# hwwang55/GraphGAN

Hardware: AMD Instinct MI355X
Metric: sampled_edges_per_sec (higher is better)
Workload: dtype f32

## Files before the change

### graphgan_amd/csrc/gg_api.hip

```cpp
#include <stdarg.h>
#include <stdlib.h>
#include <string.h>
#include <sys/stat.h>
#include <unistd.h>

#include <algorithm>
#include <atomic>
#include <thread>

#include "gg_internal.h"

namespace gg {

thread_local std::string g_last_error;

int fail(gg_ctx *ctx, int code, const char *fmt, ...) {
    char buf[1024];
    va_list ap;
    va_start(ap, fmt);
    vsnprintf(buf, sizeof(buf), fmt, ap);
    va_end(ap);
    g_last_error = buf;
    if (ctx) ctx->err = buf;
    return code;
// ... 329 lines not shown
    hipDeviceProp_t prop;
    GG_HIP(nullptr, hipGetDeviceProperties(&prop, cfg->device));
    if (strncmp(prop.gcnArchName, "gfx950", 6) != 0)
        return fail(nullptr, GG_EHIP, "gg_create: device %d is %s; kernels are built for gfx950 only", cfg->device, prop.gcnArchName);
    GG_HIP(nullptr, hipSetDevice(cfg->device));

    gg_ctx *ctx = new gg_ctx();
    ctx->n_node = n_node;
    ctx->n_emb = n_emb;
    ctx->ld = (n_emb + 3) / 4 * 4;
    ctx->cfg = *cfg;
    ctx->device = cfg->device;
    ctx->n_cus = prop.multiProcessorCount > 0 ? prop.multiProcessorCount : 256;
    if (const char *lv = getenv("GG_WALK_LEVELS")) ctx->walk_levels = atoi(lv);
    if (const char *pe = getenv("GG_PROFILE_EVERY")) ctx->profile_every = std::max(0, atoi(pe));
    if (const char *fw = getenv("GG_COMM_FAKE_WORLD")) ctx->fake_world = atoi(fw);
    if (const char *ow = getenv("GG_COMM_OWNER")) ctx->owner_exchange = atoi(ow);
    if (const char *bf = getenv("GG_COMM_BF16")) ctx->comm_bf16 = atoi(bf) != 0;
    if (const char *om = getenv("GG_COMM_OWNER_MIN")) ctx->owner_min_bound = atoll(om);
    if (const char *dt = getenv("GG_DETERMINISTIC")) ctx->deterministic = atoi(dt) != 0;
    if (const char *nc = getenv("GG_NO_DIST_CACHE")) ctx->dc_enabled = atoi(nc) == 0;
    if (const char *ft = getenv("GG_FIN_THRESHOLD")) ctx->fin_threshold = std::max(0, atoi(ft));
    if (const char *st = getenv("GG_STAGE_T")) ctx->sg_threshold = std::max(0, atoi(st));
    if (const char *ws = getenv("GG_WALK_SPLIT")) ctx->split_enabled = atoi(ws) != 0;
    if (const char *em = getenv("GG_ES_MODE")) ctx->es_mode = std::min(2, std::max(0, atoi(em)));
    if (const char *er = getenv("GG_ES_RATIO")) ctx->es_ratio_num = std::max(1, atoi(er));
    if (const char *eh = getenv("GG_ES_HUB")) ctx->es_hub = std::max(0, atoi(eh));
    if (const char *wm = getenv("GG_WALK_SPLIT_MIN")) ctx->split_min_walks = std::max(512, atoi(wm));
    for (auto &m : ctx->alive_prof) for (auto &v : m) v = -1;
    if (const char *dr = getenv("GG_COMM_DENSE_RATIO")) ctx->dense_exchange_ratio = (float)atof(dr);
#define GG_TRY(call)                        \
    do {                                    \
        int rc__ = (call);                  \
        if (rc__ != GG_OK) {                \
            g_last_error = ctx->err;        \
            gg_destroy(ctx);                \
            return rc__;                    \
        }                                   \
    } while (0)
    auto body = [&]() -> int {
        GG_HIP(ctx, hipStreamCreateWithFlags(&ctx->stream, hipStreamNonBlocking));
        {
            int lo = 0, hi = 0;
            const char *wp = getenv("GG_WALK_PRIORITY");
            if (wp && atoi(wp) != 0 && hipDeviceGetStreamPriorityRange(&lo, &hi) == hipSuccess && hi != lo)
                GG_HIP(ctx, hipStreamCreateWithPriority(&ctx->stream2, hipStreamNonBlocking, atoi(wp) > 0 ? hi : lo));
// ... 62 lines not shown
    return GG_OK;
}

int gg_destroy(gg_ctx *ctx) {
    if (!ctx) return GG_OK;
    (void)hipSetDevice(ctx->device);
    if (ctx->stream) (void)hipStreamSynchronize(ctx->stream);
    if (ctx->stream2) (void)hipStreamSynchronize(ctx->stream2);
    comm_destroy(ctx);
    for (int m = 0; m < 2; ++m) {
        Model &M = ctx->model[m];
        float *ps[] = {M.E, M.b, M.mE, M.vE, M.mb, M.vb};
        for (float *p : ps)
            if (p) (void)hipFree(p);
    }
    void *ps[] = {ctx->gradE, ctx->gradb, ctx->touched, ctx->touched_list, ctx->touched_cnt, ctx->g_rowptr, ctx->g_col, ctx->dev_ctr,
                  ctx->es, ctx->es_stamp, ctx->g_rev};
    for (void *p : ps)
        if (p) (void)hipFree(p);
    free_trees(ctx);
    DevBuf *bufs[] = {&ctx->w_slots_m[0], &ctx->w_slots_m[1], &ctx->w_ptr_m[0], &ctx->w_ptr_m[1], &ctx->w_samples, &ctx->w_paths, &ctx->w_len, &ctx->w_status,
                      &ctx->w_first, &ctx->w_abort, &ctx->w_scratch, &ctx->d_center, &ctx->d_neighbor, &ctx->d_label, &ctx->d_cnt,
                      &ctx->d_ptr, &ctx->g_node1, &ctx->g_node2, &ctx->g_reward, &ctx->g_cnt, &ctx->g_ptr, &ctx->scan_tmp,
                      &ctx->step_u, &ctx->step_v, &ctx->step_x, &ctx->sg_cnt, &ctx->sg_off, &ctx->sg_slot, &ctx->sg_list, &ctx->sg_rows, &ctx->sg_bias, &ctx->sg_tot, &ctx->sg_key, &ctx->touched_ptr, &ctx->x_cnt, &ctx->x_send_ids, &ctx->x_send_rows,
                      &ctx->x_recv_ids, &ctx->x_recv_rows, &ctx->x_nglob, &ctx->x_own, &ctx->st_item, &ctx->st_item2, &ctx->st_cur, &ctx->st_prev, &ctx->st_len,
                      &ctx->st_alive, &ctx->st_rank, &ctx->bfs_key, &ctx->bfs_bm, &ctx->bfs_misc, &ctx->bfs_sparse, &ctx->bfs_rowptr32, &ctx->lv_pfx, &ctx->dc_keys, &ctx->dc_vals, &ctx->dc_words, &ctx->lv_beg, &ctx->lv_k, &ctx->lv_chunks, &ctx->lv_coff, &ctx->lv_scores, &ctx->lv_chunk_owner, &ctx->lv_prefix, &ctx->lv_big, &ctx->lv_fe, &ctx->fin_list, &ctx->table_bad, &ctx->sgp_cnt, &ctx->sgp_off, &ctx->sgp_slot, &ctx->sgp_list, &ctx->sgp_tot, &ctx->sgp_key, &ctx->sgp_scan, &ctx->sgp_hub, &ctx->sg_hub, &ctx->hub_acc,
                      &ctx->q3_store, &ctx->q3s_off, &ctx->ep_center, &ctx->ep_neighbor, &ctx->ep_label, &ctx->ep_node1, &ctx->ep_node2, &ctx->ep_reward, &ctx->topk_adj,
                      &ctx->gs_es, &ctx->gs_cpre, &ctx->pt_starts, &ctx->pt_paths, &ctx->pt_len, &ctx->pt_cnt, &ctx->pt_ptr, &ctx->pt_noise, &ctx->pt_sample};
    for (DevBuf *b : bufs) b->release();
    for (hipEvent_t e : ctx->lv_ev)
        if (e) (void)hipEventDestroy(e);
    for (auto &tr : ctx->tm_ev)
        for (hipEvent_t e : tr)
            if (e) (void)hipEventDestroy(e);
    for (hipEvent_t e : ctx->pt_ev)
        if (e) (void)hipEventDestroy(e);
    if (ctx->h_pin) (void)hipHostFree(ctx->h_pin);
    for (hipEvent_t e : {ctx->ev_walk_done, ctx->ev_slots_done, ctx->ev_gen_pass, ctx->ev_main_mark, ctx->ev_fork, ctx->ev_join, ctx->ev_score[0], ctx->ev_score[1]})
        if (e) (void)hipEventDestroy(e);
    if (ctx->stream3) {
        (void)hipStreamSynchronize(ctx->stream3);
        (void)hipStreamDestroy(ctx->stream3);
    }
    if (ctx->stream2) {
        (void)hipStreamSynchronize(ctx->stream2);
        (void)hipStreamDestroy(ctx->stream2);
    }
// ... 673 lines not shown
```

### graphgan_amd/csrc/gg_internal.h

```cpp
#pragma once
#include <hip/hip_runtime.h>
#include <stdint.h>
#include <stdio.h>
#include <string>
#include <vector>

#include "../../include/graphgan_hip.h"

namespace gg {

struct DevBuf {
    void *p = nullptr;
    size_t bytes = 0;
    hipError_t reserve(size_t need) {
        if (need <= bytes) return hipSuccess;
        if (p) {
            (void)hipDeviceSynchronize();
            (void)hipFree(p);
        }
        p = nullptr;
        bytes = 0;
        size_t want = need + need / 4 + 256;
        hipError_t e = hipMalloc(&p, want);
        if (e == hipSuccess) bytes = want;
// ... 137 lines not shown
    gg::DevBuf d_center, d_neighbor, d_label, d_cnt, d_ptr;
    int64_t d_rows = 0;
    gg::DevBuf g_node1, g_node2, g_reward, g_cnt, g_ptr;
    int64_t g_pairs = 0;
    bool g_paths_valid = false;
    bool g_begun = false;
    struct { int32_t n_slots = 0, n_sample = 0; uint64_t seed = 0; uint32_t stream = 0; } g_begun_args;
    gg::DevBuf touched_ptr;
    gg::DevBuf bfs_key, bfs_bm, bfs_misc, bfs_sparse, bfs_rowptr32;
    bool bfs_rowptr32_valid = false;
    gg::DevBuf q3_store, q3s_off;
    int64_t q3_words = 0;
    bool q3_store_ready = false;
    gg::DevBuf ep_center, ep_neighbor, ep_label, ep_node1, ep_node2, ep_reward;
    int64_t ep_rows = 0, ep_pairs = 0;
    std::vector<int32_t> ep_slots;
    bool in_epoch_add = false;
    int n_cus = 256;
    gg::DevBuf scan_tmp, step_u, step_v, step_x;
    gg::DevBuf sg_cnt, sg_off, sg_slot, sg_list, sg_rows, sg_bias, sg_tot, sg_key;
    bool g_pairs_filled = false;
    bool sg_cnt_dirty = false;
    gg::DevBuf sgp_cnt, sgp_off, sgp_slot, sgp_list, sgp_tot, sgp_key, sgp_scan, sgp_hub;
    gg::DevBuf sg_hub, hub_acc;
    int64_t hub_cap = 0;
    hipEvent_t ev_slots_done = nullptr;
    bool g_slots_ready = false;
    bool sgp_cnt_clean = false;
    int g_slots_unused = 0;
    int64_t g_slots_walks = 0;
    int32_t g_slots_stride = 0;
    int32_t *sg_cnt_active = nullptr;
    bool sg_active = false;
    int sg_threshold = 64;

    unsigned long long *dev_ctr = nullptr;
    gg_counters ctr{};

    void *comm = nullptr;
    bool comm_rsag = true;
    size_t grad_elems_padded = 0;
    int64_t d_rows_max = 0, g_pairs_max = 0;
    int64_t step_bound = 0;
    int64_t comm_steps_sparse = 0, comm_steps_dense = 0, comm_bytes_sent = 0;
    int32_t rank = 0, world = 1;
    bool deterministic = true;
    float dense_exchange_ratio = 1.5f;
    int32_t fake_world = 0;
    gg::DevBuf x_cnt, x_send_ids, x_send_rows, x_recv_ids, x_recv_rows;
    gg::DevBuf x_nglob;
    gg::DevBuf x_own;
    int32_t owner_exchange = 1;
    bool comm_bf16 = false;
    int64_t owner_min_bound = 4096;
    int64_t comm_steps_owner = 0;

// ... 88 lines not shown
```

### graphgan_amd/csrc/steps.hip

```cpp
#include <stdlib.h>

#include <algorithm>
#include <cmath>
#include <vector>

#include "gg_internal.h"

namespace gg {

struct HubAcc {
    unsigned long long *acc;
    int64_t cap;
    float scale;
};
__device__ __forceinline__ unsigned long long *hub_row(const HubAcc &h, int slot, int ld) {
    const int64_t k = -3 - (int64_t)slot;
    return (slot <= -3 && k < h.cap) ? h.acc + k * (ld + 1) : nullptr;
}
__device__ __forceinline__ void hub_add(unsigned long long *p, float x, float scale) {
    atomicAdd(p, (unsigned long long)__float2ll_rn(x * scale));
}

struct StepArgs {
    float *E, *b;
    float *gE, *gb;
    int32_t *touched, *touched_list, *touched_cnt;
    int ld, track;
    const int32_t *u, *v;
    const float *x;
    int n;
    float lambda, inv_n;
    const int64_t *n_glob;
    int is_d;
    int ppg;
    unsigned long long *prof;
    const int32_t *slot_v, *slot_u;
    float *stage, *stage_b;
    HubAcc hub;
};

__global__ __launch_bounds__(256) void pair_occ_count_kernel(const int32_t *u, const int32_t *v, int n, int ppg, int32_t *cnt,
                                                             int32_t *slot_v, int32_t *slot_u) {
    const int p = blockIdx.x * blockDim.x + threadIdx.x;
    if (p >= n) return;
    slot_v[p] = atomicAdd(&cnt[v[p]], 1);
    const bool run_end = p == n - 1 || (p + 1) % ppg == 0 || u[p + 1] != u[p];
    slot_u[p] = run_end ? atomicAdd(&cnt[u[p]], 1) : -2;
}

__global__ __launch_bounds__(256) void pair_occ_slot_kernel(const int32_t *u, const int32_t *v, int n, const int32_t *cnt, const int32_t *off,
                                                            int T, int32_t *slot_v, int32_t *slot_u, int32_t *key) {
    const int p = blockIdx.x * blockDim.x + threadIdx.x;
    if (p >= n) return;
    const int iv = v[p], iu = u[p];
    const int sv = cnt[iv] <= T ? off[iv] + slot_v[p] : -3 - off[iv];
    slot_v[p] = sv;
    if (sv >= 0) key[sv] = 2 * p + 1;
    if (slot_u[p] != -2) {
        const int su = cnt[iu] <= T ? off[iu] + slot_u[p] : -3 - off[iu];
        slot_u[p] = su;
        if (su >= 0) key[su] = 2 * p;
    }
// ... 74 lines not shown
        for (int i = 0; i < NF; ++i) {
            const int f = t + 16 * i;
            if (f < a.ld) {
                const float x = fu[f], y = fv[f];
                accu[i] += ds * y + a.lambda * x;
                const float gval = ds * x + a.lambda * y;
                if (st) gv[f] = gval;
                else atomicAdd(gv + f, gval);
            }
        }
        if (t == 0) {
            const float gbv = a.is_d ? ds + a.lambda * bv : ds;
            if (st) {
                a.stage_b[slv] = gbv;
            } else {
                atomicAdd(a.gb + iv, gbv);
                if (a.track) a.touched[iv] = 1;
            }
        }
    }
    flush_u(p1 - 1);
}

template <int NF, bool STAGED>
__global__ __launch_bounds__(256) void pair_grad16_kernel(const StepArgs a) {
    const int t = threadIdx.x & 15;
    const int64_t g = ((int64_t)blockIdx.x * blockDim.x + threadIdx.x) >> 4;
    const int64_t p0 = g * 16;
    if (p0 >= a.n) return;
    const int np = (int)min((int64_t)16, (int64_t)a.n - p0);
    const float inv_n = a.n_glob ? 1.0f / (float)(*a.n_glob) : a.inv_n;
    const bool mine = t < np;
    const int myu = mine ? a.u[p0 + t] : 0, myv = mine ? a.v[p0 + t] : 0;
    const float myx = mine ? a.x[p0 + t] : 0.f;
    const int my_sv = (STAGED && mine) ? a.slot_v[p0 + t] : -1;
    const int my_su = (STAGED && mine) ? a.slot_u[p0 + t] : -1;
    const float mybv = a.b[myv];
    const int nextu = __shfl(myu, (t + 1) & 15, 16);
    const bool my_end = mine && (t == np - 1 || nextu != myu);
    auto fetch = [&](int j, float (&ru)[NF], float (&rv)[NF]) {
        const int jj = j < np ? j : 0;
        const float *su = a.E + (int64_t)__shfl(myu, jj, 16) * a.ld, *sv = a.E + (int64_t)__shfl(myv, jj, 16) * a.ld;
#pragma unroll
        for (int i = 0; i < NF; ++i) {
            const int f = t + 16 * i;
            const int fc = f < a.ld ? f : a.ld - 1;
            ru[i] = su[fc];
            rv[i] = sv[fc];
        }
    };
    float U[3][NF], V[3][NF], accu[NF];
#pragma unroll
    for (int i = 0; i < NF; ++i) accu[i] = 0.f;
    fetch(0, U[0], V[0]);
    fetch(1, U[1], V[1]);
#pragma unroll 1
    for (int j0 = 0; j0 < np; j0 += 3) {
#pragma unroll
        for (int r = 0; r < 3; ++r) {
            const int j = j0 + r;
            if (j >= np) break;
            fetch(j + 2, U[(r + 2) % 3], V[(r + 2) % 3]);
// ... 9 lines not shown
            acc += __shfl_xor(acc, 4, 64);
            acc += __shfl_xor(acc, 2, 64);
            acc += __shfl_xor(acc, 1, 64);
            const float bv = __shfl(mybv, j, 16), xj = __shfl(myx, j, 16);
            const float s = acc + bv;
            const float sg = 1.0f / (1.0f + expf(-s));
            float ds;
            if (a.is_d) {
                ds = sg - xj;
            } else {
                const bool inside = (sg >= 1e-5f) && (sg <= 1.0f);
                ds = inside ? -(xj * inv_n) * (1.0f - sg) : 0.0f;
            }
            const int iv = __shfl(myv, j, 16), iu = __shfl(myu, j, 16);
            const int slv = __shfl(my_sv, j, 16), slu = __shfl(my_su, j, 16);
            const bool st = STAGED && slv >= 0;
            unsigned long long *hv = STAGED && !st ? hub_row(a.hub, slv, a.ld) : nullptr;
            float *gv = st ? a.stage + (int64_t)slv * a.ld : a.gE + (int64_t)iv * a.ld;
#pragma unroll
            for (int i = 0; i < NF; ++i) {
                const int f = t + 16 * i;
                if (f < a.ld) {
                    accu[i] += ds * V[r][i] + a.lambda * U[r][i];
                    const float gval = ds * U[r][i] + a.lambda * V[r][i];
                    if (st) gv[f] = gval;
                    else if (STAGED && hv) hub_add(hv + f, gval, a.hub.scale);
                    else atomicAdd(gv + f, gval);
                }
            }
            if (t == 0) {
                const float gbv = a.is_d ? ds + a.lambda * bv : ds;
                if (st) {
                    a.stage_b[slv] = gbv;
                } else {
                    if (STAGED && hv) hub_add(hv + a.ld, gbv, a.hub.scale);
                    else atomicAdd(a.gb + iv, gbv);
                    if (a.track) a.touched[iv] = 1;
                }
            }
            if (__shfl((int)my_end, j, 16)) {
                if (STAGED && slu >= 0) {
                    float *gu = a.stage + (int64_t)slu * a.ld;
#pragma unroll
                    for (int i = 0; i < NF; ++i) {
                        const int f = t + 16 * i;
                        if (f < a.ld) gu[f] = accu[i];
                    }
                    if (t == 0) a.stage_b[slu] = 0.f;
                } else {
                    float *gu = a.gE + (int64_t)iu * a.ld;
                    unsigned long long *hu = STAGED ? hub_row(a.hub, slu, a.ld) : nullptr;
#pragma unroll
                    for (int i = 0; i < NF; ++i) {
                        const int f = t + 16 * i;
                        if (f < a.ld) {
                            if (STAGED && hu) hub_add(hu + f, accu[i], a.hub.scale);
                            else atomicAdd(gu + f, accu[i]);
                        }
                    }
                    if (t == 0 && a.track) a.touched[iu] = 1;
                }
#pragma unroll
                for (int i = 0; i < NF; ++i) accu[i] = 0.f;
            }
        }
    }
}

struct PathArgs {
    float *E, *b, *gE, *gb;
    int32_t *touched, *touched_list, *touched_cnt;
// ... 206 lines not shown
#pragma unroll
            for (int i = 0; i < NF; ++i) { R[sl][i] = R[sl + 1][i]; A[sl][i] = A[sl + 1][i]; }
        }
        enter(2, Rq[0], qnode[0], qslot[0], qbv[0]);
        qnode[0] = qnode[1]; qbv[0] = qbv[1]; qslot[0] = qslot[1];
#pragma unroll
        for (int i = 0; i < NF; ++i) Rq[0][i] = Rq[1][i];
    }
}

struct OptArgs {
    float *E, *b, *mE, *vE, *mb, *vb, *gE, *gb;
    const int64_t *touched_ptr;
    const int64_t *touched_total;
    int64_t nE;
    int n_node, ld;
    float lr_t, b1, b2, eps, lr;
    int32_t *touched, *touched_list, *touched_cnt;
    int32_t *sg_cnt;
    const int4 *sg_list;
    const int64_t *sg_tot;
    const float *stage, *stage_b;
    const int32_t *stage_key;
    unsigned long long *bad;
};

__device__ __forceinline__ bool nonfinite4(const float4 &x) { return !(__builtin_isfinite(x.x) && __builtin_isfinite(x.y) && __builtin_isfinite(x.z) && __builtin_isfinite(x.w)); }

__device__ __forceinline__ void adam_elem(float &var, float &m, float &v, float g, const OptArgs &a) {
    m = m * a.b1;
    m = m + (1.0f - a.b1) * g;
    v = v * a.b2;
    v = v + (g * g) * (1.0f - a.b2);
    var = var - (a.lr_t * m) / (sqrtf(v) + a.eps);
}

__global__ __launch_bounds__(256) void adam_dense_kernel(const OptArgs a) {
    const int64_t n4 = a.nE >> 2;
    const int64_t stride = (int64_t)gridDim.x * blockDim.x;
    const float4 z = make_float4(0.f, 0.f, 0.f, 0.f);
    bool bad = false;
    for (int64_t i = (int64_t)blockIdx.x * blockDim.x + threadIdx.x; i < n4; i += stride) {
        float4 var = ((float4 *)a.E)[i], m = ((float4 *)a.mE)[i], v = ((float4 *)a.vE)[i];
        const float4 g = ((const float4 *)a.gE)[i];
        adam_elem(var.x, m.x, v.x, g.x, a);
        adam_elem(var.y, m.y, v.y, g.y, a);
// ... 45 lines not shown
            float var = a.b[row];
            const float g = a.gb[row];
            if (SGD) {
                var -= a.lr * g;
            } else {
                float m = a.mb[row], v = a.vb[row];
                adam_elem(var, m, v, g, a);
                a.mb[row] = m;
                a.vb[row] = v;
            }
            if (!__builtin_isfinite(var)) *a.bad = 1ull;
            a.b[row] = var;
            a.gb[row] = 0.f;
            a.touched[row] = 0;
            if (a.sg_cnt) a.sg_cnt[row] = 0;
        }
    }
}

constexpr int DET_MAX_PAIRS = 256;
constexpr int DET_THREADS = 1024;
constexpr int DET_GROUPS = DET_THREADS / 16;
constexpr size_t DET_LDS_ROW_BYTES = 144 * 1024;

__device__ __forceinline__ unsigned group16_ballot(bool pred) {
    const uint64_t m = __ballot(pred);
    return (unsigned)(m >> (threadIdx.x & 48)) & 0xffffu;
}

template <int NF, bool ROWS_IN_LDS, int OPT, bool SMALLN>
__global__ __launch_bounds__(DET_THREADS) void pair_grad_det_kernel(const StepArgs a, const OptArgs o) {
    static_assert(OPT == 0 || ROWS_IN_LDS, "the fused update needs every table read in front of the barrier");
    extern __shared__ float det_rows[];
    __shared__ int32_t ids[2 * DET_MAX_PAIRS];
    __shared__ float coef[DET_MAX_PAIRS], coefb[DET_MAX_PAIRS];
    const int t = threadIdx.x & 15, g = threadIdx.x >> 4;
    const int n = a.n, ld = a.ld, nchunk = ld >> 2;
    const float inv_n = a.n_glob ? 1.0f / (float)(*a.n_glob) : a.inv_n;
    const bool stamp = a.prof && blockIdx.x == 0 && (threadIdx.x == 0 || threadIdx.x == DET_THREADS - 64);
    unsigned long long *const pw = a.prof + (threadIdx.x ? 8 : 0);
    if (stamp) pw[0] = wall_clock64();
    for (int s = threadIdx.x; s < 2 * n; s += DET_THREADS) ids[s] = s < n ? a.u[s] : a.v[s - n];
    for (int p = g; p < n; p += DET_GROUPS) {
        const int iu = a.u[p], iv = a.v[p];
        const float xp = a.x[p];
        const float bv = a.b[iv];
        const float4 *ru = (const float4 *)(a.E + (int64_t)iu * ld);
        const float4 *rv = (const float4 *)(a.E + (int64_t)iv * ld);
        float acc = 0.f;
        for (int c = t; c < nchunk; c += 16) {
            const float4 x = ru[c], y = rv[c];
// ... 226 lines not shown
    if (!det_rows_fit_lds(ctx, s)) {
        const dim3 grid(det_workgroups(s.n));
        if (s.n <= 64) hipLaunchKernelGGL((pair_grad_det_kernel<NF, false, 0, true>), grid, dim3(DET_THREADS), 0, ctx->stream, s, o);
        else hipLaunchKernelGGL((pair_grad_det_kernel<NF, false, 0, false>), grid, dim3(DET_THREADS), 0, ctx->stream, s, o);
        return hipSuccess;
    }
    if (opt == 1) return launch_pair_grad_det_lds<NF, 1>(ctx, s, o);
    if (opt == 2) return launch_pair_grad_det_lds<NF, 2>(ctx, s, o);
    return launch_pair_grad_det_lds<NF, 0>(ctx, s, o);
}

template <int SGD>
__global__ __launch_bounds__(256) void sparse_opt_kernel(const OptArgs a) {
    const int t = threadIdx.x & 15;
    const int g0 = (blockIdx.x * blockDim.x + threadIdx.x) >> 4;
    const int ng = (gridDim.x * blockDim.x) >> 4;
    const int cnt = (int)*a.touched_total;
    const int nchunk = a.ld >> 2;
    for (int r = g0; r < cnt; r += ng) opt_row<SGD>(a, a.touched_list[r], t, nchunk);
}

constexpr int STAGE_SORT = 64;

template <int MODE>
__global__ __launch_bounds__(256) void staged_opt_kernel(const OptArgs a) {
    constexpr bool SGD = MODE == 1;
    __shared__ int32_t perm_s[16][STAGE_SORT];
    const int t = threadIdx.x & 15;
    int32_t *const perm = perm_s[threadIdx.x >> 4];
    const int64_t g0 = ((int64_t)blockIdx.x * blockDim.x + threadIdx.x) >> 4, ng = ((int64_t)gridDim.x * blockDim.x) >> 4;
    const int64_t n_rows = a.sg_tot[0];
    const int nchunk = a.ld >> 2;
    for (int64_t r = g0; r < n_rows; r += ng) {
        const int4 e = a.sg_list[r];
        const int row = e.x, n = e.z;
        const float4 *const seg = (const float4 *)(a.stage + (int64_t)e.y * a.ld);
        const float *const sb = a.stage_b + e.y;
        const int32_t *const key = a.stage_key + e.y;
        float4 g[4];
#pragma unroll
        for (int i = 0; i < 4; ++i) g[i] = make_float4(0.f, 0.f, 0.f, 0.f);
        float gbias = 0.f;
        auto add_row = [&](const float4 *src) {
#pragma unroll
            for (int i = 0; i < 4; ++i) {
                const int c = t + 16 * i;
                if (c < nchunk) {
                    const float4 x = src[c];
                    g[i].x += x.x; g[i].y += x.y; g[i].z += x.z; g[i].w += x.w;
                }
            }
        };
        if (n <= STAGE_SORT) {
            if (n > 1) {
                int k[4], rk[4];
#pragma unroll
                for (int i = 0; i < 4; ++i) {
                    k[i] = (t + 16 * i < n) ? key[t + 16 * i] : 0x7fffffff;
                    rk[i] = 0;
                }
#pragma unroll
                for (int j = 0; j < 4; ++j) {
                    if (16 * j < n) {
                        const int nl = min(n - 16 * j, 16);
                        for (int l = 0; l < nl; ++l) {
                            const int kk = __shfl(k[j], l, 16);
#pragma unroll
                            for (int i = 0; i < 4; ++i) rk[i] += kk < k[i];
                        }
                    }
                }
#pragma unroll
                for (int i = 0; i < 4; ++i)
                    if (t + 16 * i < n) perm[rk[i]] = t + 16 * i;
            } else if (t == 0) {
                perm[0] = 0;
            }
            __builtin_amdgcn_fence(__ATOMIC_RELEASE, "wavefront");
            __builtin_amdgcn_wave_barrier();
            __builtin_amdgcn_fence(__ATOMIC_ACQUIRE, "wavefront");
            int o = 0;
            for (; o + 4 <= n; o += 4) {
                const float4 *s0 = seg + (int64_t)perm[o] * nchunk, *s1 = seg + (int64_t)perm[o + 1] * nchunk;
                const float4 *s2 = seg + (int64_t)perm[o + 2] * nchunk, *s3 = seg + (int64_t)perm[o + 3] * nchunk;
#pragma unroll
                for (int i = 0; i < 4; ++i) {
                    const int c = t + 16 * i;
                    if (c < nchunk) {
                        const float4 x0 = s0[c], x1 = s1[c], x2 = s2[c], x3 = s3[c];
                        g[i].x += x0.x; g[i].y += x0.y; g[i].z += x0.z; g[i].w += x0.w;
                        g[i].x += x1.x; g[i].y += x1.y; g[i].z += x1.z; g[i].w += x1.w;
                        g[i].x += x2.x; g[i].y += x2.y; g[i].z += x2.z; g[i].w += x2.w;
                        g[i].x += x3.x; g[i].y += x3.y; g[i].z += x3.z; g[i].w += x3.w;
                    }
                }
            }
            for (; o < n; ++o) add_row(seg + (int64_t)perm[o] * nchunk);
            for (int q = t; q < n; q += 16) gbias += sb[perm[q]];
            __builtin_amdgcn_wave_barrier();
        } else {
            int last = -1;
            for (int q = 0; q < n; ++q) {
                int best = 0x7fffffff, besto = 0;
                for (int o = t; o < n; o += 16) {
                    const int kk = key[o];
                    if (kk > last && kk < best) { best = kk; besto = o; }
                }
#pragma unroll
                for (int m = 8; m >= 1; m >>= 1) {
                    const int ob = __shfl_xor(best, m, 16), oo = __shfl_xor(besto, m, 16);
                    if (ob < best) { best = ob; besto = oo; }
                }
                add_row(seg + (int64_t)besto * nchunk);
                if ((q & 15) == t) gbias += sb[besto];
                last = best;
            }
        }
        gbias += __shfl_xor(gbias, 8, 64);
        gbias += __shfl_xor(gbias, 4, 64);
        gbias += __shfl_xor(gbias, 2, 64);
        gbias += __shfl_xor(gbias, 1, 64);
        const int64_t o4 = ((int64_t)row * a.ld) >> 2;
        if (MODE == 2) {
#pragma unroll
            for (int i = 0; i < 4; ++i) {
                const int c = t + 16 * i;
                if (c < nchunk) ((float4 *)a.gE)[o4 + c] = g[i];
            }
            if (t == 0) {
                a.gb[row] = gbias;
                a.touched[row] = 1;
                a.sg_cnt[row] = 0;
            }
            continue;
        }
#pragma unroll
        for (int i = 0; i < 4; ++i) {
            const int c = t + 16 * i;
            if (c >= nchunk) continue;
            float4 var = ((float4 *)a.E)[o4 + c];
            if (SGD) {
                var.x -= a.lr * g[i].x; var.y -= a.lr * g[i].y; var.z -= a.lr * g[i].z; var.w -= a.lr * g[i].w;
            } else {
                float4 m = ((float4 *)a.mE)[o4 + c], v = ((float4 *)a.vE)[o4 + c];
                adam_elem(var.x, m.x, v.x, g[i].x, a);
                adam_elem(var.y, m.y, v.y, g[i].y, a);
                adam_elem(var.z, m.z, v.z, g[i].z, a);
                adam_elem(var.w, m.w, v.w, g[i].w, a);
                ((float4 *)a.mE)[o4 + c] = m;
                ((float4 *)a.vE)[o4 + c] = v;
            }
            if (nonfinite4(var)) *a.bad = 1ull;
            ((float4 *)a.E)[o4 + c] = var;
        }
        if (t == 0) {
            float var = a.b[row];
            if (SGD) {
                var -= a.lr * gbias;
            } else {
                float m = a.mb[row], v = a.vb[row];
                adam_elem(var, m, v, gbias, a);
                a.mb[row] = m;
                a.vb[row] = v;
// ... 159 lines not shown
    GG_HIP(ctx, ctx->sg_list.reserve(sizeof(int4) * (size_t)ctx->n_node));
    GG_HIP(ctx, ctx->sg_slot.reserve(sizeof(int32_t) * (size_t)n_occ));
    GG_HIP(ctx, ctx->sg_bias.reserve(sizeof(float) * (size_t)n_stage));
    GG_HIP(ctx, ctx->sg_key.reserve(sizeof(int32_t) * (size_t)n_stage));
    GG_HIP(ctx, ctx->sg_tot.reserve(sizeof(int64_t) * 4));
    {
        const int64_t cap = std::min<int64_t>(ctx->n_node, n_occ / ((int64_t)ctx->sg_threshold + 1) + 1);
        const size_t before = ctx->hub_acc.bytes;
        if (ctx->hub_acc.reserve(sizeof(unsigned long long) * (size_t)cap * (ctx->ld + 1)) != hipSuccess) {
            (void)hipGetLastError();
            ctx->hub_cap = 0;
            return 1;
        }
        if (ctx->hub_acc.bytes != before || was_dirty) GG_HIP(ctx, hipMemsetAsync(ctx->hub_acc.p, 0, ctx->hub_acc.bytes, ctx->stream));
        ctx->hub_cap = (int64_t)(ctx->hub_acc.bytes / (sizeof(unsigned long long) * (ctx->ld + 1)));
    }
    if (ctx->sg_rows.reserve(sizeof(float) * (size_t)n_stage * ctx->ld) != hipSuccess) {
        (void)hipGetLastError();
        return 1;
    }
    return GG_OK;
}

static int staged_finish(gg_ctx *ctx, int which, int64_t n, int64_t n_occ, bool early_index = false) {
    const int opt = ctx->cfg.optimizer;
    OptArgs o = make_opt_args(ctx, which);
    DevBuf &b_cnt = early_index ? ctx->sgp_cnt : ctx->sg_cnt, &b_list = early_index ? ctx->sgp_list : ctx->sg_list;
    DevBuf &b_tot = early_index ? ctx->sgp_tot : ctx->sg_tot, &b_key = early_index ? ctx->sgp_key : ctx->sg_key;
    o.sg_cnt = b_cnt.as<int32_t>(); o.sg_list = b_list.as<int4>(); o.sg_tot = b_tot.as<int64_t>();
    o.stage = ctx->sg_rows.as<float>(); o.stage_b = ctx->sg_bias.as<float>(); o.stage_key = b_key.as<int32_t>();
    int nb = cdiv((int64_t)std::min<int64_t>(n_occ, ctx->n_node) * 16, 256);
    if (nb > 4096) nb = 4096;
    if (nb < 1) nb = 1;
    const bool replicas = ctx->comm || ctx->fake_world > 1;
    if (replicas) hipLaunchKernelGGL(staged_opt_kernel<2>, dim3(nb), dim3(256), 0, ctx->stream, o);
    else if (opt == GG_OPT_SGD) hipLaunchKernelGGL(staged_opt_kernel<1>, dim3(nb), dim3(256), 0, ctx->stream, o);
    else hipLaunchKernelGGL(staged_opt_kernel<0>, dim3(nb), dim3(256), 0, ctx->stream, o);
    ctx->sg_active = true;
    ctx->sg_cnt_active = o.sg_cnt;
    const int rc = apply_optimizer(ctx, which, n);
    ctx->sg_active = false;
    if (rc != GG_OK) return rc;
    if (!replicas)
        hipLaunchKernelGGL(add_word_kernel, dim3(1), dim3(1), 0, ctx->stream, ctx->touched_ptr.as<int64_t>() + ctx->n_node, b_tot.as<int64_t>());
    GG_HIP(ctx, hipGetLastError());
    if (early_index) ctx->sgp_cnt_clean = true;
    else ctx->sg_cnt_dirty = false;
    return GG_OK;
}

static bool staged_allowed(const gg_ctx *ctx) {
    return ctx->sg_threshold > 0 && ctx->ld <= 256 && ctx->cfg.optimizer != GG_OPT_ADAM_DENSE && !getenv("GG_NO_STAGED_GRAD");
}

int run_step(gg_ctx *ctx, int which, const int32_t *d_u, const int32_t *d_v, const float *d_x, int32_t n) {
    if (n <= 0) return GG_OK;
    Model &M = ctx->model[which];
    const int opt = ctx->cfg.optimizer;
    StepArgs s{};
    s.E = M.E; s.b = M.b; s.gE = ctx->gradE; s.gb = ctx->gradb;
// ... 50 lines not shown
    const int groups = cdiv(n, s.ppg);
    const int blocks = cdiv((int64_t)groups * 16, 256);
    const int nf = (ctx->ld + 15) / 16;
    bool staged = n >= 16384 && n < (1 << 30) && staged_allowed(ctx);
    if (staged) {
        int rc = staged_reserve(ctx, 2 * (int64_t)n, 2 * (int64_t)n);
        if (rc < 0) return rc;
        if (rc == 1) staged = false;
    }
    if (staged) {
        int rc;
        int32_t *cnt = ctx->sg_cnt.as<int32_t>(), *off = ctx->sg_off.as<int32_t>(), *slot_v = ctx->sg_slot.as<int32_t>(), *slot_u = slot_v + n;
        hipLaunchKernelGGL(pair_occ_count_kernel, dim3(cdiv(n, 256)), dim3(256), 0, ctx->stream, d_u, d_v, n, s.ppg, cnt, slot_v, slot_u);
        rc = device_segment_rows(ctx, cnt, ctx->n_node, ctx->sg_threshold, off, ctx->sg_list.as<int4>(), ctx->sg_tot.as<int64_t>());
        if (rc != GG_OK) return rc;
        rc = hub_index(ctx, cnt, off, ctx->sg_hub, ctx->sg_tot.as<int64_t>(), ctx->stream);
        if (rc != GG_OK) return rc;
        hipLaunchKernelGGL(pair_occ_slot_kernel, dim3(cdiv(n, 256)), dim3(256), 0, ctx->stream, d_u, d_v, n, cnt, off, ctx->sg_threshold, slot_v, slot_u,
                           ctx->sg_key.as<int32_t>());
        s.slot_v = slot_v; s.slot_u = slot_u;
        s.stage = ctx->sg_rows.as<float>(); s.stage_b = ctx->sg_bias.as<float>();
        const float scale = hub_scale(!s.is_d, n);
        s.hub = hub_args(ctx, scale);
        if (nf <= 4) hipLaunchKernelGGL((pair_grad16_kernel<4, true>), dim3(blocks), dim3(256), 0, ctx->stream, s);
        else if (nf <= 8) hipLaunchKernelGGL((pair_grad16_kernel<8, true>), dim3(blocks), dim3(256), 0, ctx->stream, s);
        else hipLaunchKernelGGL((pair_grad16_kernel<16, true>), dim3(blocks), dim3(256), 0, ctx->stream, s);
        hub_finalize(ctx, false, scale, s.gE, s.gb);
        if (ctx->tm_cur >= 0) GG_HIP(ctx, hipEventRecord(ctx->tm_ev[ctx->tm_cur][1], ctx->stream));
        return staged_finish(ctx, which, n, 2 * (int64_t)n);
    }
    if (s.ppg == PAIRS_PER_GROUP && nf <= 16 && !getenv("GG_OLD_PAIR_GRAD")) {
        if (nf <= 4) hipLaunchKernelGGL((pair_grad16_kernel<4, false>), dim3(blocks), dim3(256), 0, ctx->stream, s);
        else if (nf <= 8) hipLaunchKernelGGL((pair_grad16_kernel<8, false>), dim3(blocks), dim3(256), 0, ctx->stream, s);
        else hipLaunchKernelGGL((pair_grad16_kernel<16, false>), dim3(blocks), dim3(256), 0, ctx->stream, s);
    } else if (nf <= 4) hipLaunchKernelGGL((pair_grad_kernel<4, false>), dim3(blocks), dim3(256), 0, ctx->stream, s);
    else if (nf <= 8) hipLaunchKernelGGL((pair_grad_kernel<8, false>), dim3(blocks), dim3(256), 0, ctx->stream, s);
    else if (nf <= 16) hipLaunchKernelGGL((pair_grad_kernel<16, false>), dim3(blocks), dim3(256), 0, ctx->stream, s);
    else hipLaunchKernelGGL((pair_grad_kernel<32, false>), dim3(blocks), dim3(256), 0, ctx->stream, s);
    if (ctx->tm_cur >= 0) GG_HIP(ctx, hipEventRecord(ctx->tm_ev[ctx->tm_cur][1], ctx->stream));

    return apply_optimizer(ctx, which, n);
}

template <bool STAGED>
static void launch_path_grad(gg_ctx *ctx, const PathArgs &p, int blocks, int nf) {
    const dim3 g(blocks), b(256);
    if (p.stride <= 17) {
        if (nf <= 4) hipLaunchKernelGGL((path_grad_kernel<4, STAGED, true>), g, b, 0, ctx->stream, p);
        else if (nf <= 8) hipLaunchKernelGGL((path_grad_kernel<8, STAGED, true>), g, b, 0, ctx->stream, p);
        else hipLaunchKernelGGL((path_grad_kernel<16, STAGED, true>), g, b, 0, ctx->stream, p);
    } else {
        if (nf <= 4) hipLaunchKernelGGL((path_grad_kernel<4, STAGED, false>), g, b, 0, ctx->stream, p);
// ... 591 lines not shown
```

Measured before the change: 652.9 million.

## Stage scalar coefficients and source-row snapshots instead of per-pair gradient rows

In the staged pair-gradient path, the kernel no longer writes a full gradient row for each v-occurrence. It now stores the scalar coefficient ds plus a signed index to a snapshot of the matching u row, written once per u-run. The staged optimizer kernel rebuilds each v gradient as ds*U + lambda*V from the snapshot and the row's own embedding. For small ld it uses a narrower register variant that holds the embedding row, plus a waves-per-EU hint and 32-bit loop indices. This cuts staging write bandwidth in exchange for indirect reads and extra arithmetic in the optimizer pass. The new path is on by default, and GG_STAGE_PAIR_ROWS restores the old behaviour.

```diff
diff --git a/graphgan_amd/csrc/gg_api.hip b/graphgan_amd/csrc/gg_api.hip
--- a/graphgan_amd/csrc/gg_api.hip
+++ b/graphgan_amd/csrc/gg_api.hip
@@ -375,6 +375,7 @@
     if (const char *nc = getenv("GG_NO_DIST_CACHE")) ctx->dc_enabled = atoi(nc) == 0;
     if (const char *ft = getenv("GG_FIN_THRESHOLD")) ctx->fin_threshold = std::max(0, atoi(ft));
     if (const char *st = getenv("GG_STAGE_T")) ctx->sg_threshold = std::max(0, atoi(st));
+    if (const char *pr = getenv("GG_STAGE_PAIR_ROWS")) ctx->stage_pair_rows = atoi(pr) != 0;
     if (const char *ws = getenv("GG_WALK_SPLIT")) ctx->split_enabled = atoi(ws) != 0;
     if (const char *em = getenv("GG_ES_MODE")) ctx->es_mode = std::min(2, std::max(0, atoi(em)));
     if (const char *er = getenv("GG_ES_RATIO")) ctx->es_ratio_num = std::max(1, atoi(er));
@@ -483,7 +484,7 @@
     DevBuf *bufs[] = {&ctx->w_slots_m[0], &ctx->w_slots_m[1], &ctx->w_ptr_m[0], &ctx->w_ptr_m[1], &ctx->w_samples, &ctx->w_paths, &ctx->w_len, &ctx->w_status,
                       &ctx->w_first, &ctx->w_abort, &ctx->w_scratch, &ctx->d_center, &ctx->d_neighbor, &ctx->d_label, &ctx->d_cnt,
                       &ctx->d_ptr, &ctx->g_node1, &ctx->g_node2, &ctx->g_reward, &ctx->g_cnt, &ctx->g_ptr, &ctx->scan_tmp,
-                      &ctx->step_u, &ctx->step_v, &ctx->step_x, &ctx->sg_cnt, &ctx->sg_off, &ctx->sg_slot, &ctx->sg_list, &ctx->sg_rows, &ctx->sg_bias, &ctx->sg_tot, &ctx->sg_key, &ctx->touched_ptr, &ctx->x_cnt, &ctx->x_send_ids, &ctx->x_send_rows,
+                      &ctx->step_u, &ctx->step_v, &ctx->step_x, &ctx->sg_cnt, &ctx->sg_off, &ctx->sg_slot, &ctx->sg_list, &ctx->sg_rows, &ctx->sg_bias, &ctx->sg_tot, &ctx->sg_key, &ctx->sg_coef, &ctx->touched_ptr, &ctx->x_cnt, &ctx->x_send_ids, &ctx->x_send_rows,
                       &ctx->x_recv_ids, &ctx->x_recv_rows, &ctx->x_nglob, &ctx->x_own, &ctx->st_item, &ctx->st_item2, &ctx->st_cur, &ctx->st_prev, &ctx->st_len,
                       &ctx->st_alive, &ctx->st_rank, &ctx->bfs_key, &ctx->bfs_bm, &ctx->bfs_misc, &ctx->bfs_sparse, &ctx->bfs_rowptr32, &ctx->lv_pfx, &ctx->dc_keys, &ctx->dc_vals, &ctx->dc_words, &ctx->lv_beg, &ctx->lv_k, &ctx->lv_chunks, &ctx->lv_coff, &ctx->lv_scores, &ctx->lv_chunk_owner, &ctx->lv_prefix, &ctx->lv_big, &ctx->lv_fe, &ctx->fin_list, &ctx->table_bad, &ctx->sgp_cnt, &ctx->sgp_off, &ctx->sgp_slot, &ctx->sgp_list, &ctx->sgp_tot, &ctx->sgp_key, &ctx->sgp_scan, &ctx->sgp_hub, &ctx->sg_hub, &ctx->hub_acc,
                       &ctx->q3_store, &ctx->q3s_off, &ctx->ep_center, &ctx->ep_neighbor, &ctx->ep_label, &ctx->ep_node1, &ctx->ep_node2, &ctx->ep_reward, &ctx->topk_adj,
diff --git a/graphgan_amd/csrc/gg_internal.h b/graphgan_amd/csrc/gg_internal.h
--- a/graphgan_amd/csrc/gg_internal.h
+++ b/graphgan_amd/csrc/gg_internal.h
@@ -183,6 +183,7 @@
     bool g_pairs_filled = false;
     bool sg_cnt_dirty = false;
     gg::DevBuf sgp_cnt, sgp_off, sgp_slot, sgp_list, sgp_tot, sgp_key, sgp_scan, sgp_hub;
+    gg::DevBuf sg_coef;
     gg::DevBuf sg_hub, hub_acc;
     int64_t hub_cap = 0;
     hipEvent_t ev_slots_done = nullptr;
@@ -193,6 +194,7 @@
     int32_t g_slots_stride = 0;
     int32_t *sg_cnt_active = nullptr;
     bool sg_active = false;
+    bool stage_pair_rows = false;
     int sg_threshold = 64;
 
     unsigned long long *dev_ctr = nullptr;
diff --git a/graphgan_amd/csrc/steps.hip b/graphgan_amd/csrc/steps.hip
--- a/graphgan_amd/csrc/steps.hip
+++ b/graphgan_amd/csrc/steps.hip
@@ -2,6 +2,7 @@
 
 #include <algorithm>
 #include <cmath>
+#include <type_traits>
 #include <vector>
 
 #include "gg_internal.h"
@@ -37,7 +38,14 @@
     const int32_t *slot_v, *slot_u;
     float *stage, *stage_b;
     HubAcc hub;
+    int32_t *coef_src;
+    int64_t snap0;
 };
+
+__device__ __forceinline__ unsigned group16_ballot(bool pred) {
+    const uint64_t m = __ballot(pred);
+    return (unsigned)(m >> (threadIdx.x & 48)) & 0xffffu;
+}
 
 __global__ __launch_bounds__(256) void pair_occ_count_kernel(const int32_t *u, const int32_t *v, int n, int ppg, int32_t *cnt,
                                                              int32_t *slot_v, int32_t *slot_u) {
@@ -158,8 +166,9 @@
     flush_u(p1 - 1);
 }
 
-template <int NF, bool STAGED>
+template <int NF, bool STAGED, bool COEF = false>
 __global__ __launch_bounds__(256) void pair_grad16_kernel(const StepArgs a) {
+    static_assert(STAGED || !COEF, "coefficients are staged");
     const int t = threadIdx.x & 15;
     const int64_t g = ((int64_t)blockIdx.x * blockDim.x + threadIdx.x) >> 4;
     const int64_t p0 = g * 16;
@@ -174,6 +183,7 @@
     const float mybv = a.b[myv];
     const int nextu = __shfl(myu, (t + 1) & 15, 16);
     const bool my_end = mine && (t == np - 1 || nextu != myu);
+    const unsigned ends = COEF ? group16_ballot(my_end) : 0u;
     auto fetch = [&](int j, float (&ru)[NF], float (&rv)[NF]) {
         const int jj = j < np ? j : 0;
         const float *su = a.E + (int64_t)__shfl(myu, jj, 16) * a.ld, *sv = a.E + (int64_t)__shfl(myv, jj, 16) * a.ld;
@@ -229,6 +239,7 @@
                 const int f = t + 16 * i;
                 if (f < a.ld) {
                     accu[i] += ds * V[r][i] + a.lambda * U[r][i];
+                    if (COEF && st) continue;
                     const float gval = ds * U[r][i] + a.lambda * V[r][i];
                     if (st) gv[f] = gval;
                     else if (STAGED && hv) hub_add(hv + f, gval, a.hub.scale);
@@ -238,7 +249,8 @@
             if (t == 0) {
                 const float gbv = a.is_d ? ds + a.lambda * bv : ds;
                 if (st) {
-                    a.stage_b[slv] = gbv;
+                    a.stage_b[slv] = COEF ? ds : gbv;
+                    if (COEF) a.coef_src[slv] = ~(int32_t)(a.snap0 + p0 + j + __builtin_ctz(ends >> j));
                 } else {
                     if (STAGED && hv) hub_add(hv + a.ld, gbv, a.hub.scale);
                     else atomicAdd(a.gb + iv, gbv);
@@ -246,14 +258,25 @@
                 }
             }
             if (__shfl((int)my_end, j, 16)) {
+                if (COEF) {
+                    float *sn = a.stage + (a.snap0 + p0 + j) * a.ld;
+#pragma unroll
+                    for (int i = 0; i < NF; ++i) {
+                        const int f = t + 16 * i;
+                        if (f < a.ld) sn[f] = U[r][i];
+                    }
+                }
                 if (STAGED && slu >= 0) {
-                    float *gu = a.stage + (int64_t)slu * a.ld;
+                    float *gu = a.stage + (COEF ? p0 + j : (int64_t)slu) * a.ld;
 #pragma unroll
                     for (int i = 0; i < NF; ++i) {
                         const int f = t + 16 * i;
                         if (f < a.ld) gu[f] = accu[i];
                     }
-                    if (t == 0) a.stage_b[slu] = 0.f;
+                    if (t == 0) {
+                        a.stage_b[slu] = 0.f;
+                        if (COEF) a.coef_src[slu] = (int32_t)(p0 + j);
+                    }
                 } else {
                     float *gu = a.gE + (int64_t)iu * a.ld;
                     unsigned long long *hu = STAGED ? hub_row(a.hub, slu, a.ld) : nullptr;
@@ -506,6 +529,9 @@
     const int64_t *sg_tot;
     const float *stage, *stage_b;
     const int32_t *stage_key;
+    const int32_t *coef_src;
+    float lambda;
+    int is_d;
     unsigned long long *bad;
 };
 
@@ -597,11 +623,6 @@
 constexpr int DET_THREADS = 1024;
 constexpr int DET_GROUPS = DET_THREADS / 16;
 constexpr size_t DET_LDS_ROW_BYTES = 144 * 1024;
-
-__device__ __forceinline__ unsigned group16_ballot(bool pred) {
-    const uint64_t m = __ballot(pred);
-    return (unsigned)(m >> (threadIdx.x & 48)) & 0xffffu;
-}
 
 template <int NF, bool ROWS_IN_LDS, int OPT, bool SMALLN>
 __global__ __launch_bounds__(DET_THREADS) void pair_grad_det_kernel(const StepArgs a, const OptArgs o) {
@@ -874,28 +895,41 @@
 
 constexpr int STAGE_SORT = 64;
 
-template <int MODE>
-__global__ __launch_bounds__(256) void staged_opt_kernel(const OptArgs a) {
+template <int MODE, bool COEF = false, int NC = 4>
+__global__ __launch_bounds__(256) __attribute__((amdgpu_waves_per_eu(COEF && MODE == 0 ? 5 : 1))) void staged_opt_kernel(const OptArgs a) {
     constexpr bool SGD = MODE == 1;
-    __shared__ int32_t perm_s[16][STAGE_SORT];
+    __shared__ int32_t perm_s[COEF ? 1 : 16][COEF ? 1 : STAGE_SORT];
+    __shared__ int2 ent_s[COEF ? 16 : 1][COEF ? STAGE_SORT : 1];
     const int t = threadIdx.x & 15;
-    int32_t *const perm = perm_s[threadIdx.x >> 4];
-    const int64_t g0 = ((int64_t)blockIdx.x * blockDim.x + threadIdx.x) >> 4, ng = ((int64_t)gridDim.x * blockDim.x) >> 4;
-    const int64_t n_rows = a.sg_tot[0];
+    int32_t *const perm = perm_s[COEF ? 0 : threadIdx.x >> 4];
+    int2 *const ent = ent_s[COEF ? threadIdx.x >> 4 : 0];
+    using idx_t = std::conditional_t<COEF, int32_t, int64_t>;
+    const idx_t g0 = (idx_t)(((int64_t)blockIdx.x * blockDim.x + threadIdx.x) >> 4), ng = (idx_t)(((int64_t)gridDim.x * blockDim.x) >> 4);
+    const idx_t n_rows = (idx_t)a.sg_tot[0];
     const int nchunk = a.ld >> 2;
-    for (int64_t r = g0; r < n_rows; r += ng) {
+    for (idx_t r = g0; r < n_rows; r += ng) {
         const int4 e = a.sg_list[r];
         const int row = e.x, n = e.z;
         const float4 *const seg = (const float4 *)(a.stage + (int64_t)e.y * a.ld);
         const float *const sb = a.stage_b + e.y;
         const int32_t *const key = a.stage_key + e.y;
-        float4 g[4];
-#pragma unroll
-        for (int i = 0; i < 4; ++i) g[i] = make_float4(0.f, 0.f, 0.f, 0.f);
+        const int32_t *const csrc = COEF ? a.coef_src + e.y : nullptr;
+        auto bias_term = [&](int32_t s, float d, float bown) { return s < 0 && a.is_d ? d + a.lambda * bown : d; };
+        float4 g[NC];
+#pragma unroll
+        for (int i = 0; i < NC; ++i) g[i] = make_float4(0.f, 0.f, 0.f, 0.f);
         float gbias = 0.f;
+        const int64_t o4 = ((int64_t)row * a.ld) >> 2;
+        constexpr bool HOLD = COEF && NC <= 2;
+        float4 var0[HOLD ? NC : 1];
+        if (HOLD) {
+#pragma unroll
+            for (int i = 0; i < NC; ++i)
+                if (t + 16 * i < nchunk) var0[i] = ((const float4 *)a.E)[o4 + t + 16 * i];
+        }
         auto add_row = [&](const float4 *src) {
 #pragma unroll
-            for (int i = 0; i < 4; ++i) {
+            for (int i = 0; i < NC; ++i) {
                 const int c = t + 16 * i;
                 if (c < nchunk) {
                     const float4 x = src[c];
@@ -903,6 +937,21 @@
                 }
             }
         };
+        auto term = [&](float4 &gs, const float4 &x, bool odd, float d, const float4 &vr) {
+            gs.x += odd ? d * x.x + a.lambda * vr.x : x.x;
+            gs.y += odd ? d * x.y + a.lambda * vr.y : x.y;
+            gs.z += odd ? d * x.z + a.lambda * vr.z : x.z;
+            gs.w += odd ? d * x.w + a.lambda * vr.w : x.w;
+        };
+        auto add_entry = [&](int32_t s, float d) {
+            const bool odd = s < 0;
+            const float4 *const r4 = (const float4 *)a.stage + (int64_t)(odd ? ~s : s) * nchunk;
+#pragma unroll
+            for (int i = 0; i < NC; ++i) {
+                const int c = t + 16 * i;
+                if (c < nchunk) term(g[i], r4[c], odd, d, HOLD ? var0[HOLD ? i : 0] : ((const float4 *)a.E)[o4 + c]);
+            }
+        };
         if (n <= STAGE_SORT) {
             if (n > 1) {
                 int k[4], rk[4];
@@ -924,31 +973,58 @@
                 }
 #pragma unroll
                 for (int i = 0; i < 4; ++i)
-                    if (t + 16 * i < n) perm[rk[i]] = t + 16 * i;
+                    if (t + 16 * i < n) {
+                        if (COEF) ent[rk[i]] = make_int2(csrc[t + 16 * i], __float_as_int(sb[t + 16 * i]));
+                        else perm[rk[i]] = t + 16 * i;
+                    }
             } else if (t == 0) {
-                perm[0] = 0;
+                if (COEF) ent[0] = make_int2(csrc[0], __float_as_int(sb[0]));
+                else perm[0] = 0;
             }
             __builtin_amdgcn_fence(__ATOMIC_RELEASE, "wavefront");
             __builtin_amdgcn_wave_barrier();
             __builtin_amdgcn_fence(__ATOMIC_ACQUIRE, "wavefront");
             int o = 0;
-            for (; o + 4 <= n; o += 4) {
-                const float4 *s0 = seg + (int64_t)perm[o] * nchunk, *s1 = seg + (int64_t)perm[o + 1] * nchunk;
-                const float4 *s2 = seg + (int64_t)perm[o + 2] * nchunk, *s3 = seg + (int64_t)perm[o + 3] * nchunk;
-#pragma unroll
-                for (int i = 0; i < 4; ++i) {
-                    const int c = t + 16 * i;
-                    if (c < nchunk) {
-                        const float4 x0 = s0[c], x1 = s1[c], x2 = s2[c], x3 = s3[c];
-                        g[i].x += x0.x; g[i].y += x0.y; g[i].z += x0.z; g[i].w += x0.w;
-                        g[i].x += x1.x; g[i].y += x1.y; g[i].z += x1.z; g[i].w += x1.w;
-                        g[i].x += x2.x; g[i].y += x2.y; g[i].z += x2.z; g[i].w += x2.w;
-                        g[i].x += x3.x; g[i].y += x3.y; g[i].z += x3.z; g[i].w += x3.w;
+            if (COEF) {
+                const float4 *const st4 = (const float4 *)a.stage;
+                for (; o + 4 <= n; o += 4) {
+                    const int2 e0 = ent[o], e1 = ent[o + 1], e2 = ent[o + 2], e3 = ent[o + 3];
+#pragma unroll
+                    for (int i = 0; i < NC; ++i) {
+                        const int c = t + 16 * i;
+                        if (c < nchunk) {
+                            const float4 x0 = st4[(int64_t)(e0.x < 0 ? ~e0.x : e0.x) * nchunk + c], x1 = st4[(int64_t)(e1.x < 0 ? ~e1.x : e1.x) * nchunk + c];
+                            const float4 x2 = st4[(int64_t)(e2.x < 0 ? ~e2.x : e2.x) * nchunk + c], x3 = st4[(int64_t)(e3.x < 0 ? ~e3.x : e3.x) * nchunk + c];
+                            const float4 vr = HOLD ? var0[HOLD ? i : 0] : ((const float4 *)a.E)[o4 + c];
+                            term(g[i], x0, e0.x < 0, __int_as_float(e0.y), vr);
+                            term(g[i], x1, e1.x < 0, __int_as_float(e1.y), vr);
+                            term(g[i], x2, e2.x < 0, __int_as_float(e2.y), vr);
+                            term(g[i], x3, e3.x < 0, __int_as_float(e3.y), vr);
+                        }
                     }
                 }
-            }
-            for (; o < n; ++o) add_row(seg + (int64_t)perm[o] * nchunk);
-            for (int q = t; q < n; q += 16) gbias += sb[perm[q]];
+                for (; o < n; ++o) add_entry(ent[o].x, __int_as_float(ent[o].y));
+                const float bown = a.b[row];
+                for (int q = t; q < n; q += 16) gbias += bias_term(ent[q].x, __int_as_float(ent[q].y), bown);
+            } else {
+                for (; o + 4 <= n; o += 4) {
+                    const float4 *s0 = seg + (int64_t)perm[o] * nchunk, *s1 = seg + (int64_t)perm[o + 1] * nchunk;
+                    const float4 *s2 = seg + (int64_t)perm[o + 2] * nchunk, *s3 = seg + (int64_t)perm[o + 3] * nchunk;
+#pragma unroll
+                    for (int i = 0; i < NC; ++i) {
+                        const int c = t + 16 * i;
+                        if (c < nchunk) {
+                            const float4 x0 = s0[c], x1 = s1[c], x2 = s2[c], x3 = s3[c];
+                            g[i].x += x0.x; g[i].y += x0.y; g[i].z += x0.z; g[i].w += x0.w;
+                            g[i].x += x1.x; g[i].y += x1.y; g[i].z += x1.z; g[i].w += x1.w;
+                            g[i].x += x2.x; g[i].y += x2.y; g[i].z += x2.z; g[i].w += x2.w;
+                            g[i].x += x3.x; g[i].y += x3.y; g[i].z += x3.z; g[i].w += x3.w;
+                        }
+                    }
+                }
+                for (; o < n; ++o) add_row(seg + (int64_t)perm[o] * nchunk);
+                for (int q = t; q < n; q += 16) gbias += sb[perm[q]];
+            }
             __builtin_amdgcn_wave_barrier();
         } else {
             int last = -1;
@@ -963,8 +1039,9 @@
                     const int ob = __shfl_xor(best, m, 16), oo = __shfl_xor(besto, m, 16);
                     if (ob < best) { best = ob; besto = oo; }
                 }
-                add_row(seg + (int64_t)besto * nchunk);
-                if ((q & 15) == t) gbias += sb[besto];
+                if (COEF) add_entry(csrc[besto], sb[besto]);
+                else add_row(seg + (int64_t)besto * nchunk);
+                if ((q & 15) == t) gbias += COEF ? bias_term(csrc[besto], sb[besto], a.b[row]) : sb[besto];
                 last = best;
             }
         }
@@ -972,10 +1049,9 @@
         gbias += __shfl_xor(gbias, 4, 64);
         gbias += __shfl_xor(gbias, 2, 64);
         gbias += __shfl_xor(gbias, 1, 64);
-        const int64_t o4 = ((int64_t)row * a.ld) >> 2;
         if (MODE == 2) {
 #pragma unroll
-            for (int i = 0; i < 4; ++i) {
+            for (int i = 0; i < NC; ++i) {
                 const int c = t + 16 * i;
                 if (c < nchunk) ((float4 *)a.gE)[o4 + c] = g[i];
             }
@@ -987,10 +1063,10 @@
             continue;
         }
 #pragma unroll
-        for (int i = 0; i < 4; ++i) {
+        for (int i = 0; i < NC; ++i) {
             const int c = t + 16 * i;
             if (c >= nchunk) continue;
-            float4 var = ((float4 *)a.E)[o4 + c];
+            float4 var = HOLD ? var0[HOLD ? i : 0] : ((float4 *)a.E)[o4 + c];
             if (SGD) {
                 var.x -= a.lr * g[i].x; var.y -= a.lr * g[i].y; var.z -= a.lr * g[i].z; var.w -= a.lr * g[i].w;
             } else {
@@ -1196,7 +1272,14 @@
     return GG_OK;
 }
 
-static int staged_finish(gg_ctx *ctx, int which, int64_t n, int64_t n_occ, bool early_index = false) {
+template <int MODE>
+static void launch_staged_opt(gg_ctx *ctx, const OptArgs &o, int nb, bool coef) {
+    if (coef && o.ld <= 128) hipLaunchKernelGGL((staged_opt_kernel<MODE, true, 2>), dim3(nb), dim3(256), 0, ctx->stream, o);
+    else if (coef) hipLaunchKernelGGL((staged_opt_kernel<MODE, true>), dim3(nb), dim3(256), 0, ctx->stream, o);
+    else hipLaunchKernelGGL((staged_opt_kernel<MODE, false>), dim3(nb), dim3(256), 0, ctx->stream, o);
+}
+
+static int staged_finish(gg_ctx *ctx, int which, int64_t n, int64_t n_occ, bool early_index = false, bool coef = false) {
     const int opt = ctx->cfg.optimizer;
     OptArgs o = make_opt_args(ctx, which);
     DevBuf &b_cnt = early_index ? ctx->sgp_cnt : ctx->sg_cnt, &b_list = early_index ? ctx->sgp_list : ctx->sg_list;
@@ -1207,9 +1290,10 @@
     if (nb > 4096) nb = 4096;
     if (nb < 1) nb = 1;
     const bool replicas = ctx->comm || ctx->fake_world > 1;
-    if (replicas) hipLaunchKernelGGL(staged_opt_kernel<2>, dim3(nb), dim3(256), 0, ctx->stream, o);
-    else if (opt == GG_OPT_SGD) hipLaunchKernelGGL(staged_opt_kernel<1>, dim3(nb), dim3(256), 0, ctx->stream, o);
-    else hipLaunchKernelGGL(staged_opt_kernel<0>, dim3(nb), dim3(256), 0, ctx->stream, o);
+    if (coef) { o.coef_src = ctx->sg_coef.as<int32_t>(); o.lambda = ctx->model[which].lambda; o.is_d = which == 1; }
+    if (replicas) launch_staged_opt<2>(ctx, o, nb, coef);
+    else if (opt == GG_OPT_SGD) launch_staged_opt<1>(ctx, o, nb, coef);
+    else launch_staged_opt<0>(ctx, o, nb, coef);
     ctx->sg_active = true;
     ctx->sg_cnt_active = o.sg_cnt;
     const int rc = apply_optimizer(ctx, which, n);
@@ -1306,12 +1390,22 @@
         s.stage = ctx->sg_rows.as<float>(); s.stage_b = ctx->sg_bias.as<float>();
         const float scale = hub_scale(!s.is_d, n);
         s.hub = hub_args(ctx, scale);
-        if (nf <= 4) hipLaunchKernelGGL((pair_grad16_kernel<4, true>), dim3(blocks), dim3(256), 0, ctx->stream, s);
-        else if (nf <= 8) hipLaunchKernelGGL((pair_grad16_kernel<8, true>), dim3(blocks), dim3(256), 0, ctx->stream, s);
-        else hipLaunchKernelGGL((pair_grad16_kernel<16, true>), dim3(blocks), dim3(256), 0, ctx->stream, s);
+        const bool coef = !ctx->stage_pair_rows;
+        if (coef) {
+            GG_HIP(ctx, ctx->sg_coef.reserve(sizeof(int32_t) * 2 * (size_t)n));
+            s.coef_src = ctx->sg_coef.as<int32_t>(); s.snap0 = n;
+        }
+        const dim3 grid(blocks), block(256);
+        if (coef) {
+            if (nf <= 4) hipLaunchKernelGGL((pair_grad16_kernel<4, true, true>), grid, block, 0, ctx->stream, s);
+            else if (nf <= 8) hipLaunchKernelGGL((pair_grad16_kernel<8, true, true>), grid, block, 0, ctx->stream, s);
+            else hipLaunchKernelGGL((pair_grad16_kernel<16, true, true>), grid, block, 0, ctx->stream, s);
+        } else if (nf <= 4) hipLaunchKernelGGL((pair_grad16_kernel<4, true>), grid, block, 0, ctx->stream, s);
+        else if (nf <= 8) hipLaunchKernelGGL((pair_grad16_kernel<8, true>), grid, block, 0, ctx->stream, s);
+        else hipLaunchKernelGGL((pair_grad16_kernel<16, true>), grid, block, 0, ctx->stream, s);
         hub_finalize(ctx, false, scale, s.gE, s.gb);
         if (ctx->tm_cur >= 0) GG_HIP(ctx, hipEventRecord(ctx->tm_ev[ctx->tm_cur][1], ctx->stream));
-        return staged_finish(ctx, which, n, 2 * (int64_t)n);
+        return staged_finish(ctx, which, n, 2 * (int64_t)n, false, coef);
     }
     if (s.ppg == PAIRS_PER_GROUP && nf <= 16 && !getenv("GG_OLD_PAIR_GRAD")) {
         if (nf <= 4) hipLaunchKernelGGL((pair_grad16_kernel<4, false>), dim3(blocks), dim3(256), 0, ctx->stream, s);
```

After: 659.0 million, median of 6. No clear change (+0.9%).
